# Aedelon/ProteinBERT-PyTorch-Replication

Measured on AMD Instinct MI355X. Metric: sequences/sec (whole node) ProteinBERT pretrain L=512 at 1/2/4/8 MI355X, higher is better.
Workload: dtype bf16; 1 GPU; global_batch=2048, per_gpu_batch=2048, seq_len=512, parallelism=dp1, impl=hip, hip_graph=False

## Files before the change

proteinbert_pytorch_replication_amd/ops/csrc/ln.hip:

```cpp
#include "mfma.h"
#include <stdlib.h>

using namespace pbx;
typedef unsigned short bf16_t;

namespace {
constexpr int CH = 128;
constexpr int BML = 32;

__device__ __forceinline__ void load_f8(const float* p, float* v) {
  const float4 a = *reinterpret_cast<const float4*>(p);
  const float4 c = *reinterpret_cast<const float4*>(p + 4);
  v[0] = a.x; v[1] = a.y; v[2] = a.z; v[3] = a.w; v[4] = c.x; v[5] = c.y; v[6] = c.z; v[7] = c.w;
}

__device__ __forceinline__ void stage_weight(unsigned char* dst, const bf16_t* __restrict__ w, int rows) {
  stage_chunks(
      rows * 16, [&](int idx) { return *reinterpret_cast<const uint4*>(w + (size_t)idx * 8); },
      [&](int idx, uint4 v) { *reinterpret_cast<uint4*>(dst + swz256(idx >> 4, idx & 15)) = v; });
}

constexpr int PB = 32;
constexpr int YS = CH + 4;

__device__ __forceinline__ uint4 ldq(const bf16_t* p, bool ok) {
  return ok ? *reinterpret_cast<const uint4*>(p) : make_uint4(0u, 0u, 0u, 0u);
}

__device__ __forceinline__ void sample_stats(float* sh, const float* __restrict__ st, int T, int BM, int L, float eps,
                                             const float* __restrict__ sums, int Ts, float inv_n) {
  if (threadIdx.x == 0) {
    float mean, rstd;
    ln_stats(st, T, BM, L, CH, eps, mean, rstd);
    sh[0] = mean;
    sh[1] = rstd;
    if (sums != nullptr) {
      float m1, m2;
      ln_bwd_consts(sums, Ts, inv_n, m1, m2);
      sh[2] = m1;
      sh[3] = m2;
    }
  }
}

__global__ void __launch_bounds__(512) ln_linear_fwd_kernel(
    const bf16_t* __restrict__ s1, const float* __restrict__ st1, int T1, int BM1, const float* __restrict__ g1,
    const float* __restrict__ be1, const bf16_t* __restrict__ wl, const float* __restrict__ bl,
    bf16_t* __restrict__ pre_l, bf16_t* __restrict__ s2, float* __restrict__ st2, int B, int L, float eps) {
  extern __shared__ __attribute__((aligned(16))) unsigned char smem[];
  unsigned char* ws = smem;
  unsigned char* ht = smem + 32768;
  float* yt = reinterpret_cast<float*>(smem + 32768 + PB * 256);
  float* tab = yt + PB * YS;
  const int tid = threadIdx.x, lane = tid & 63, w = tid >> 6;
  const int r = lane & 31, h = lane >> 5;
  const int j = tid >> 4, ch = tid & 15;
  const int l0 = blockIdx.x * PB, l = l0 + j;
  const bool okl = l < L;
  const int TP = (L + PB - 1) / PB;
  const int nbg = gridDim.y;
  const int b0 = (int)((long)B * blockIdx.y / nbg), b1 = (int)((long)B * (blockIdx.y + 1) / nbg);
  const int nb = b1 - b0;
  float* part = tab + 2 * nb;
  stage_weight(ws, wl, CH);
  for (int i = w; i < nb; i += 8) {
    float mean, rstd;
    wave_ln_stats(st1 + (size_t)(b0 + i) * T1 * 2, T1, BM1, L, CH, eps, mean, rstd);
    if (lane == 0) {
      tab[2 * i] = mean;
      tab[2 * i + 1] = rstd;
    }
  }
  float gam[8] = {0, 0, 0, 0, 0, 0, 0, 0}, bet[8] = {0, 0, 0, 0, 0, 0, 0, 0}, bb[8];
  if (okl) {
    load_f8(g1 + (size_t)l * CH + ch * 8, gam);
    load_f8(be1 + (size_t)l * CH + ch * 8, bet);
  }
  load_f8(bl + ch * 8, bb);
  uint4 nxt = ldq(s1 + ((size_t)b0 * L + l) * CH + ch * 8, okl && nb > 0);
  __syncthreads();
  for (int b = b0; b < b1; ++b) {
    const int i = b - b0;
    const float mean = tab[2 * i], rstd = tab[2 * i + 1];
    float sv[8], h1[8];
    unpack8(nxt, sv);
#pragma unroll
    for (int e = 0; e < 8; ++e) h1[e] = okl ? (sv[e] - mean) * rstd * gam[e] + bet[e] : 0.f;
    *reinterpret_cast<uint4*>(ht + swz256(j, ch)) = packq8(h1);
    __syncthreads();
    nxt = ldq(s1 + ((size_t)(b + 1) * L + l) * CH + ch * 8, okl && b + 1 < b1);
    if (w < 4) {
      f32x16_t acc = zero16();
#pragma unroll
      for (int kk = 0; kk < 8; ++kk)
        acc = mfma32(lds_frag(ws, swz256(w * 32 + r, kk * 2 + h)), lds_frag(ht, swz256(r, kk * 2 + h)), acc);
#pragma unroll
      for (int g = 0; g < 4; ++g)
        *reinterpret_cast<float4*>(yt + r * YS + w * 32 + 8 * g + 4 * h) =
            make_float4(acc[4 * g], acc[4 * g + 1], acc[4 * g + 2], acc[4 * g + 3]);
    }
    __syncthreads();
    float pre[8], o[8];
    const float4 ya = *reinterpret_cast<const float4*>(yt + j * YS + ch * 8);
    const float4 yb = *reinterpret_cast<const float4*>(yt + j * YS + ch * 8 + 4);
    const float yv[8] = {ya.x, ya.y, ya.z, ya.w, yb.x, yb.y, yb.z, yb.w};
#pragma unroll
    for (int e = 0; e < 8; ++e) pre[e] = yv[e] + bb[e];
    f32x2 gg[4];
    {
      const f32x2 xi[4] = {(f32x2){pre[0], pre[1]}, (f32x2){pre[2], pre[3]}, (f32x2){pre[4], pre[5]},
                           (f32x2){pre[6], pre[7]}};
      gelu2_fast_n<4, false>(xi, gg);
    }
#pragma unroll
    for (int e = 0; e < 8; ++e) o[e] = h1[e] + ((e & 1) ? gg[e >> 1].y : gg[e >> 1].x);
    const uint4 oq = packq8(o);
    if (okl) {
      const size_t off = ((size_t)b * L + l) * CH + ch * 8;
      if (pre_l != nullptr) *reinterpret_cast<uint4*>(pre_l + off) = packq8(pre);
      *reinterpret_cast<uint4*>(s2 + off) = oq;
    }
    float orr[8];
    unpack8(oq, orr);
    float sa = 0.f, sq = 0.f;
#pragma unroll
    for (int e = 0; e < 8; ++e) {
      sa += orr[e];
      sq += orr[e] * orr[e];
    }
    sa = wave_reduce_sum(okl ? sa : 0.f);
    sq = wave_reduce_sum(okl ? sq : 0.f);
    if (lane == 0) { part[(i * 8 + w) * 2] = sa; part[(i * 8 + w) * 2 + 1] = sq; }
  }
  __syncthreads();
  const int vrows = min(PB, L - l0);
  for (int i = tid; i < nb; i += 512) {
    float sa = 0.f, sq = 0.f;
#pragma unroll
    for (int ww = 0; ww < 8; ++ww) {
      sa += part[(i * 8 + ww) * 2];
      sq += part[(i * 8 + ww) * 2 + 1];
    }
    const float m = sa / (float)(vrows * CH);
    st2[((size_t)(b0 + i) * TP + blockIdx.x) * 2] = m;
    st2[((size_t)(b0 + i) * TP + blockIdx.x) * 2 + 1] = fmaxf(sq - sa * m, 0.f);
  }
}

__global__ void __launch_bounds__(256) ln2_consts_kernel(const float* __restrict__ st2, int T2, int BM2,
                                                         const float* __restrict__ sums2, int TS2,
                                                         const float* __restrict__ st1, int T1, int BM1,
                                                         float* __restrict__ consts, float* __restrict__ zero128,
                                                         int B, int L, float eps) {
  const int b = blockIdx.x * 4 + (threadIdx.x >> 6);
  if (b >= B) return;
  if (zero128 != nullptr)
    *reinterpret_cast<float2*>(zero128 + (size_t)b * CH + 2 * (threadIdx.x & 63)) = make_float2(0.f, 0.f);
  float mean2, rstd2, m1, m2, mean1, rstd1;
  wave_ln_stats(st2 + (size_t)b * T2 * 2, T2, BM2, L, CH, eps, mean2, rstd2);
  wave_bwd_consts(sums2 + (size_t)b * TS2 * 2, TS2, 1.0f / (float)(L * CH), m1, m2);
  wave_ln_stats(st1 + (size_t)b * T1 * 2, T1, BM1, L, CH, eps, mean1, rstd1);
  if ((threadIdx.x & 63) == 0) {
    float4* c = reinterpret_cast<float4*>(consts + (size_t)b * 8);
    c[0] = make_float4(mean2, rstd2, m1, m2);
    c[1] = make_float4(mean1, rstd1, 0.f, 0.f);
  }
}

__global__ void __launch_bounds__(512) ln2_linear_bwd_kernel(
    const bf16_t* __restrict__ dh2, const bf16_t* __restrict__ s2, const float* __restrict__ g2,
    const bf16_t* __restrict__ pre_l, const bf16_t* __restrict__ s1,
    const float* __restrict__ g1, const float* __restrict__ be1, const bf16_t* __restrict__ wl,
    const float* __restrict__ consts,
    bf16_t* __restrict__ dh1, float* __restrict__ sums1, float* __restrict__ dg2, float* __restrict__ db2,
    float* __restrict__ dg1, float* __restrict__ db1, float* __restrict__ dwl, float* __restrict__ dbl,
    float* __restrict__ dwl_slab, float* __restrict__ dbl_slab, int B, int L) {
  extern __shared__ __attribute__((aligned(16))) unsigned char smem[];
  unsigned char* ws = smem;
  unsigned char* dt = smem + 32768;
  unsigned char* ht = dt + 32 * 256;
  float* yt = reinterpret_cast<float*>(ht + 32 * 256);
  const int tid = threadIdx.x, lane = tid & 63, w = tid >> 6;
  const int r = lane & 31, h = lane >> 5;
  const int q = tr_q(lane), tc = tr_c(lane);
  const int j = tid >> 4, ch = tid & 15;
  const int TS1 = (L + 1) / 2;
  const int nsplit = gridDim.y;
  const int b0 = (int)((long)B * blockIdx.y / nsplit), b1 = (int)((long)B * (blockIdx.y + 1) / nsplit);
  stage_weight(ws, wl, CH);
  float adbl[8] = {0, 0, 0, 0, 0, 0, 0, 0};
  f32x16_t aw0 = zero16(), aw1 = zero16();
  const int wco = (w >> 1) * 32, wci = (w & 1) * 64;
  for (int pair = blockIdx.x; pair < TS1; pair += gridDim.x) {
    const int l = pair * 2 + (j & 1);
    const bool okl = l < L;
    float ga2[8] = {0, 0, 0, 0, 0, 0, 0, 0}, ga1[8] = {0, 0, 0, 0, 0, 0, 0, 0}, bt1[8] = {0, 0, 0, 0, 0, 0, 0, 0};
    if (okl) {
      load_f8(g2 + (size_t)l * CH + ch * 8, ga2);
      load_f8(g1 + (size_t)l * CH + ch * 8, ga1);
      load_f8(be1 + (size_t)l * CH + ch * 8, bt1);
    }
    float adg2[8] = {0, 0, 0, 0, 0, 0, 0, 0}, adb2[8] = {0, 0, 0, 0, 0, 0, 0, 0};
    float adg1[8] = {0, 0, 0, 0, 0, 0, 0, 0}, adb1[8] = {0, 0, 0, 0, 0, 0, 0, 0};
    const size_t coff = (size_t)l * CH + ch * 8;
    int bs = b0 + (j >> 1);
    bool ok = okl && bs < b1;
    size_t off = (size_t)bs * L * CH + coff;
    uint4 n_dh = ldq(dh2 + off, ok), n_s2 = ldq(s2 + off, ok), n_s1 = ldq(s1 + off, ok);
    uint4 n_pr = ldq(pre_l + off, ok);
    float4 n_c0 = make_float4(0.f, 1.f, 0.f, 0.f), n_c1 = make_float4(0.f, 1.f, 0.f, 0.f);
    if (bs < b1) {
      n_c0 = *reinterpret_cast<const float4*>(consts + (size_t)bs * 8);
      n_c1 = *reinterpret_cast<const float4*>(consts + (size_t)bs * 8 + 4);
    }
    for (int bc = b0; bc < b1; bc += 16) {
      const int bcur = bs;
      const bool okc = ok;
      const size_t offc = off;
      const float mean2 = n_c0.x, rstd2 = n_c0.y, m1 = n_c0.z, m2 = n_c0.w, mean1 = n_c1.x, rstd1 = n_c1.y;
      float dh[8], sv2[8], pr[8], sv1[8], ds2[8], dp[8], xh1[8], hv[8];
      unpack8(n_dh, dh);
      unpack8(n_s2, sv2);
      unpack8(n_s1, sv1);
#pragma unroll
      for (int e = 0; e < 8; ++e) {
        const float xh2 = (sv2[e] - mean2) * rstd2;
        adg2[e] += okc ? dh[e] * xh2 : 0.f;
        adb2[e] += okc ? dh[e] : 0.f;
        ds2[e] = okc ? rstd2 * (dh[e] * ga2[e] - m1 - xh2 * m2) : 0.f;
        xh1[e] = (sv1[e] - mean1) * rstd1;
        hv[e] = okc ? xh1[e] * ga1[e] + bt1[e] : 0.f;
      }
      *reinterpret_cast<uint4*>(ht + swz256(j, ch)) = packq8(hv);
      auto prefetch = [&]() {
        bs = bc + 16 + (j >> 1);
        ok = okl && bs < b1;
        off = (size_t)bs * L * CH + coff;
        n_dh = ldq(dh2 + off, ok);
        n_s2 = ldq(s2 + off, ok);
        n_pr = ldq(pre_l + off, ok);
        n_s1 = ldq(s1 + off, ok);
        if (bs < b1) {
          n_c0 = *reinterpret_cast<const float4*>(consts + (size_t)bs * 8);
          n_c1 = *reinterpret_cast<const float4*>(consts + (size_t)bs * 8 + 4);
        }
      };
      unpack8(n_pr, pr);
      float gp[8];
      {
        const f32x2 xi[4] = {(f32x2){pr[0], pr[1]}, (f32x2){pr[2], pr[3]}, (f32x2){pr[4], pr[5]},
                             (f32x2){pr[6], pr[7]}};
        f32x2 go[4];
        gelu2_fast_n<4, true>(xi, go);
#pragma unroll
        for (int e = 0; e < 4; ++e) {
          gp[2 * e] = go[e].x;
          gp[2 * e + 1] = go[e].y;
        }
      }
#pragma unroll
      for (int e = 0; e < 8; ++e) dp[e] = ds2[e] * gp[e];
      const uint4 dq = packq8(dp);
      *reinterpret_cast<uint4*>(dt + swz256(j, ch)) = dq;
      {
        float dpr[8];
        unpack8(dq, dpr);
#pragma unroll
        for (int e = 0; e < 8; ++e) adbl[e] += dpr[e];
      }
      __syncthreads();
      prefetch();
      if (w < 4) {
        f32x16_t acc = zero16();
#pragma unroll
        for (int kk = 0; kk < 8; ++kk) {
          const int rlo = kk * 16 + 8 * h + q;
          const int col = w * 32 + tc;
          const bf16x8 fa = cat_tr(lds_tr(ws, swz256e(rlo, col)), lds_tr(ws, swz256e(rlo + 4, col)));
          acc = mfma32(fa, lds_frag(dt, swz256(r, kk * 2 + h)), acc);
        }
#pragma unroll
        for (int g = 0; g < 4; ++g)
          *reinterpret_cast<float4*>(yt + r * YS + w * 32 + 8 * g + 4 * h) =
              make_float4(acc[4 * g], acc[4 * g + 1], acc[4 * g + 2], acc[4 * g + 3]);
      }
#pragma unroll
      for (int ks = 0; ks < 2; ++ks) {
        const int rlo = ks * 16 + 8 * h + q;
        const bf16x8 fa = cat_tr(lds_tr(dt, swz256e(rlo, wco + tc)), lds_tr(dt, swz256e(rlo + 4, wco + tc)));
        const bf16x8 fb0 = cat_tr(lds_tr(ht, swz256e(rlo, wci + tc)), lds_tr(ht, swz256e(rlo + 4, wci + tc)));
        const bf16x8 fb1 =
            cat_tr(lds_tr(ht, swz256e(rlo, wci + 32 + tc)), lds_tr(ht, swz256e(rlo + 4, wci + 32 + tc)));
        aw0 = mfma32(fa, fb0, aw0);
        aw1 = mfma32(fa, fb1, aw1);
      }
      __syncthreads();
      const float4 ya = *reinterpret_cast<const float4*>(yt + j * YS + ch * 8);
      const float4 yb = *reinterpret_cast<const float4*>(yt + j * YS + ch * 8 + 4);
      const float yv[8] = {ya.x, ya.y, ya.z, ya.w, yb.x, yb.y, yb.z, yb.w};
      float o[8], sa = 0.f, sc = 0.f;
#pragma unroll
      for (int e = 0; e < 8; ++e) {
        o[e] = okc ? bfround(ds2[e] + yv[e]) : 0.f;
        const float dxh = o[e] * ga1[e];
        sa += dxh;
        sc += dxh * xh1[e];
        adg1[e] += o[e] * xh1[e];
        adb1[e] += o[e];
      }
      if (okc) *reinterpret_cast<uint4*>(dh1 + offc) = packq8(o);
#pragma unroll
      for (int m = 1; m <= 16; m <<= 1) {
        sa += __shfl_xor(sa, m, 64);
        sc += __shfl_xor(sc, m, 64);
      }
      if ((lane & 31) == 0 && bcur < b1) {
        sums1[((size_t)bcur * TS1 + pair) * 2] = sa;
        sums1[((size_t)bcur * TS1 + pair) * 2 + 1] = sc;
      }
    }
    const int l0 = pair * 2;
    float* accs[4] = {adg2, adb2, adg1, adb1};
    float* dsts[4] = {dg2, db2, dg1, db1};
#pragma unroll
    for (int a = 0; a < 4; ++a) {
      __syncthreads();
#pragma unroll
      for (int e = 0; e < 8; ++e) yt[j * CH + ch * 8 + e] = accs[a][e];
      __syncthreads();
      if (tid < 2 * CH) {
        const int par = tid >> 7, c = tid & (CH - 1);
        float v = 0.f;
#pragma unroll
        for (int k = 0; k < 16; ++k) v += yt[(2 * k + par) * CH + c];
        if (l0 + par < L) atomicAdd(dsts[a] + (size_t)(l0 + par) * CH + c, v);
      }
    }
    __syncthreads();
  }
  __syncthreads();
#pragma unroll
  for (int e = 0; e < 8; ++e) yt[j * CH + ch * 8 + e] = adbl[e];
  __syncthreads();
  if (tid < CH) {
    float a = 0.f;
#pragma unroll 8
    for (int k = 0; k < 32; ++k) a += yt[k * CH + tid];
    if (dbl_slab != nullptr) dbl_slab[(size_t)(blockIdx.y * gridDim.x + blockIdx.x) * CH + tid] = a;
    else atomicAdd(dbl + tid, a);
  }
  float* dw = dwl_slab != nullptr ? dwl_slab + (size_t)(blockIdx.y * gridDim.x + blockIdx.x) * CH * CH : dwl;
#pragma unroll
  for (int i = 0; i < 16; ++i) {
    const int co = wco + (i & 3) + 8 * (i >> 2) + 4 * h;
    if (dwl_slab != nullptr) {
      dw[(size_t)co * CH + wci + r] = aw0[i];
      dw[(size_t)co * CH + wci + 32 + r] = aw1[i];
    } else {
      atomicAdd(dw + (size_t)co * CH + wci + r, aw0[i]);
      atomicAdd(dw + (size_t)co * CH + wci + 32 + r, aw1[i]);
    }
  }
}

__global__ void __launch_bounds__(512) ln1_finalize_kernel(
    const bf16_t* __restrict__ dh1, const bf16_t* __restrict__ s1, const float* __restrict__ st1, int T1, int BM1,
    const float* __restrict__ sums1, int TS1, const float* __restrict__ g1, bf16_t* __restrict__ ds1,
    float* __restrict__ dgb, int B, int L, float eps) {
  extern __shared__ __attribute__((aligned(16))) unsigned char smem[];
  float* red = reinterpret_cast<float*>(smem);
  float* tab = red + 2 * PB * CH;
  const int tid = threadIdx.x, lane = tid & 63, w = tid >> 6;
  const int j = tid >> 4, ch = tid & 15;
  const int nbg = gridDim.y;
  const int b0 = (int)((long)B * blockIdx.y / nbg), b1 = (int)((long)B * (blockIdx.y + 1) / nbg);
  const int nb = b1 - b0;
  float* dacc = tab + 4 * nb;
  const float inv_n = 1.0f / (float)(L * CH);
  for (int i = w; i < nb; i += 8) {
    float mean, rstd, m1, m2;
    wave_ln_stats(st1 + (size_t)(b0 + i) * T1 * 2, T1, BM1, L, CH, eps, mean, rstd);
    wave_bwd_consts(sums1 + (size_t)(b0 + i) * TS1 * 2, TS1, inv_n, m1, m2);
    if (lane == 0) { tab[4 * i] = mean; tab[4 * i + 1] = rstd; tab[4 * i + 2] = m1; tab[4 * i + 3] = m2; }
  }
  for (int i = tid; i < nb * CH; i += 512) dacc[i] = 0.f;
  const int TP = (L + PB - 1) / PB;
  int it = 0;
  for (int px = blockIdx.x; px < TP; px += gridDim.x) {
    const int l = px * PB + j;
    const bool okl = l < L;
    float ga[8] = {0, 0, 0, 0, 0, 0, 0, 0};
    if (okl) load_f8(g1 + (size_t)l * CH + ch * 8, ga);
    const size_t coff = (size_t)min(l, L - 1) * CH + ch * 8;
    uint4 n_dh = *reinterpret_cast<const uint4*>(dh1 + (size_t)min(b0, B - 1) * L * CH + coff);
    uint4 n_s = *reinterpret_cast<const uint4*>(s1 + (size_t)min(b0, B - 1) * L * CH + coff);
    __syncthreads();
    for (int b = b0; b < b1; ++b, ++it) {
      const float* tb = tab + 4 * (b - b0);
      const float mean = tb[0], rstd = tb[1], m1 = tb[2], m2 = tb[3];
      float* rb = red + (it & 1) * PB * CH;
      float dv[8], sv[8], o[8];
      unpack8(n_dh, dv);
      unpack8(n_s, sv);
      const size_t noff = (size_t)min(b + 1, B - 1) * L * CH + coff;
      n_dh = *reinterpret_cast<const uint4*>(dh1 + noff);
      n_s = *reinterpret_cast<const uint4*>(s1 + noff);
#pragma unroll
      for (int e = 0; e < 8; ++e) o[e] = okl ? rstd * (dv[e] * ga[e] - m1 - (sv[e] - mean) * rstd * m2) : 0.f;
      const uint4 qv = packq8(o);
      if (okl) *reinterpret_cast<uint4*>(ds1 + (size_t)b * L * CH + (size_t)l * CH + ch * 8) = qv;
      unpack8(qv, o);
#pragma unroll
      for (int e = 0; e < 8; ++e) {
        o[e] += __shfl_xor(o[e], 16, 64);
        o[e] += __shfl_xor(o[e], 32, 64);
      }
      if (lane < 16) {
        *reinterpret_cast<float4*>(rb + w * CH + ch * 8) = make_float4(o[0], o[1], o[2], o[3]);
        *reinterpret_cast<float4*>(rb + w * CH + ch * 8 + 4) = make_float4(o[4], o[5], o[6], o[7]);
      }
      __syncthreads();
      if (tid < CH) {
        float a = 0.f;
#pragma unroll
        for (int k = 0; k < 8; ++k) a += rb[k * CH + tid];
        dacc[(b - b0) * CH + tid] += a;
      }
    }
  }
  __syncthreads();
  for (int i = tid; i < nb * CH; i += 512) atomicAdd(dgb + (size_t)(b0 + i / CH) * CH + i % CH, dacc[i]);
}

__global__ void __launch_bounds__(256) embed_fwd_kernel(const long long* __restrict__ tok, const float* __restrict__ E,
                                                        bf16_t* __restrict__ out, long rows) {
  const long i = (long)blockIdx.x * 256 + threadIdx.x;
  if (i >= rows * 16) return;
  const long row = i >> 4;
  const int c8 = (int)(i & 15);
  const long long t = tok[row];
  float v[8];
  load_f8(E + (size_t)t * CH + c8 * 8, v);
  *reinterpret_cast<uint4*>(out + row * CH + c8 * 8) = packq8(v);
}

template <bool DPRE>
__global__ void __launch_bounds__(256) embed_bwd_kernel(const long long* __restrict__ tok,
                                                        const bf16_t* __restrict__ dout, float* __restrict__ dE,
                                                        long rows, int V, float* __restrict__ slab,
                                                        const bf16_t* __restrict__ gdn, const bf16_t* __restrict__ gdw,
                                                        bf16_t* __restrict__ dpn, bf16_t* __restrict__ dpw) {
  __shared__ __attribute__((aligned(16))) unsigned char ds[256 * 256];
  __shared__ int ts[256];
  const int tid = threadIdx.x, lane = tid & 63, w = tid >> 6;
  const int r = lane & 31, h = lane >> 5;
  const int q = tr_q(lane), tc = tr_c(lane);
  const long per = (rows + gridDim.x - 1) / gridDim.x;
  const long r0 = (long)blockIdx.x * per, r1 = min(rows, r0 + per);
  f32x16_t acc = zero16();
  for (long t0 = r0; t0 < r1; t0 += 256) {
    const int n = (int)min((long)256, r1 - t0);
    __syncthreads();
    if constexpr (DPRE) {
      for (int base = tid; base < 256 * 16; base += 4 * 256) {
        uint4 gq[4], nq[4], wq[4];
#pragma unroll
        for (int i = 0; i < 4; ++i) {
          const int idx = base + i * 256, row = idx >> 4;
          const size_t off = (size_t)(t0 + min(row, n - 1)) * CH + (idx & 15) * 8;
          gq[i] = *reinterpret_cast<const uint4*>(dout + off);
          nq[i] = *reinterpret_cast<const uint4*>(gdn + off);
          wq[i] = *reinterpret_cast<const uint4*>(gdw + off);
        }
#pragma unroll
        for (int i = 0; i < 4; ++i) {
          const int idx = base + i * 256, row = idx >> 4;
          const bool ok = row < n;
          *reinterpret_cast<uint4*>(ds + swz256(row, idx & 15)) = ok ? gq[i] : make_uint4(0u, 0u, 0u, 0u);
          if (ok) {
            float g[8], pn[8], pw[8], on[8], ow[8];
            unpack8(gq[i], g);
            unpack8(nq[i], pn);
            unpack8(wq[i], pw);
#pragma unroll
            for (int e = 0; e < 8; ++e) {
              on[e] = pn[e] * g[e];
              ow[e] = pw[e] * g[e];
            }
            const size_t off = (size_t)(t0 + row) * CH + (idx & 15) * 8;
            *reinterpret_cast<uint4*>(dpn + off) = packq8(on);
            *reinterpret_cast<uint4*>(dpw + off) = packq8(ow);
          }
        }
      }
    } else {
      stage_chunks(
          256 * 16,
          [&](int idx) {
            const int row = idx >> 4;
            return row < n ? *reinterpret_cast<const uint4*>(dout + (t0 + row) * CH + (idx & 15) * 8)
                           : make_uint4(0u, 0u, 0u, 0u);
          },
          [&](int idx, uint4 v) { *reinterpret_cast<uint4*>(ds + swz256(idx >> 4, idx & 15)) = v; });
    }
    ts[tid] = tid < n ? (int)tok[t0 + tid] : -1;
    __syncthreads();
    const int colb = w * 32 + tc;
#pragma unroll 4
    for (int kb = 0; kb < 16; ++kb) {
      typedef __attribute__((ext_vector_type(8))) unsigned short u16x8;
      u16x8 oh;
#pragma unroll
      for (int j = 0; j < 8; ++j) oh[j] = ts[kb * 16 + 8 * h + j] == r ? (unsigned short)0x3F80 : (unsigned short)0;
      const int rb = kb * 16 + 8 * h + q;
      const bf16x8 fb = cat_tr(lds_tr(ds, swz256e(rb, colb)), lds_tr(ds, swz256e(rb + 4, colb)));
      acc = mfma32(__builtin_bit_cast(bf16x8, oh), fb, acc);
    }
  }
#pragma unroll
  for (int i = 0; i < 16; ++i) {
    const int v = (i & 3) + 8 * (i >> 2) + 4 * h;
    if (slab != nullptr) {
      if (v < V) slab[((size_t)blockIdx.x * V + v) * CH + w * 32 + r] = acc[i];
    } else if (v < V && acc[i] != 0.f) {
      atomicAdd(dE + v * CH + w * 32 + r, acc[i]);
    }
  }
}

int g_cus = -1;
int num_cus() {
  if (g_cus < 0) {
    int dev = 0;
    g_cus = 256;
    if (hipGetDevice(&dev) == hipSuccess) {
      hipDeviceProp_t p;
      if (hipGetDeviceProperties(&p, dev) == hipSuccess) g_cus = p.multiProcessorCount;
    }
  }
  return g_cus;
}
int persistent_grid(int tiles, int per_cu) {
  const int cap = num_cus() * per_cu;
  return tiles < cap ? (tiles > 0 ? tiles : 1) : cap;
}
}

extern "C" int pbx_colsum_add(const float* src, int rows, int cols, float* dst, const float* scale, hipStream_t st);

static bool ln_attrs_set = false;
static void set_ln_attrs() {
  if (ln_attrs_set) return;
  (void)hipFuncSetAttribute((const void*)ln_linear_fwd_kernel, hipFuncAttributeMaxDynamicSharedMemorySize, 163840);
  (void)hipFuncSetAttribute((const void*)ln2_linear_bwd_kernel, hipFuncAttributeMaxDynamicSharedMemorySize, 163840);
  (void)hipFuncSetAttribute((const void*)ln1_finalize_kernel, hipFuncAttributeMaxDynamicSharedMemorySize, 163840);
  ln_attrs_set = true;
}

static int ln_groups(int B, int L) {
  const int tp = (L + PB - 1) / PB;
  int g = (2 * num_cus() + tp - 1) / tp;
  return g < 1 ? 1 : (g > B ? B : g);
}

PBX_EXPORT int pbx_ln_linear_fwd(const void* s1, const float* st1, int T1, int BM1, const float* g1,
                                 const float* be1, const void* wl, const float* bl, void* pre_l, void* s2,
                                 float* st2, int B, int L, float eps, hipStream_t st) {
  dim3 grid((L + PB - 1) / PB, ln_groups(B, L));
  const int nbmax = (B + (int)grid.y - 1) / (int)grid.y;
  const int lds = 32768 + PB * 256 + PB * YS * 4 + nbmax * 18 * 4;
  if (lds > 163840) return (int)hipErrorInvalidValue;
  set_ln_attrs();
  hipLaunchKernelGGL(ln_linear_fwd_kernel, grid, dim3(512), lds, st, (const bf16_t*)s1, st1, T1, BM1, g1, be1,
                     (const bf16_t*)wl, bl, (bf16_t*)pre_l, (bf16_t*)s2, st2, B, L, eps);
  return pbx_launch_status();
}

static void ln2_bwd_grid(int B, int L, int det, int& gx, int& nsplit) {
  const int pairs = (L + 1) / 2;
  const int target = num_cus();
  nsplit = (target + pairs - 1) / pairs;
  if (nsplit > (B + 15) / 16) nsplit = (B + 15) / 16;
  if (nsplit < 1 || det) nsplit = 1;
  gx = pairs < target ? pairs : target;
}

PBX_EXPORT int pbx_ln2_bwd_slab_rows(int B, int L, int det) {
  int gx, nsplit;
  ln2_bwd_grid(B, L, det, gx, nsplit);
  return gx * nsplit;
}

PBX_EXPORT int pbx_ln2_linear_bwd(const void* dh2, const void* s2, const float* st2, const float* sums2, int TS2,
                                  const float* g2, const void* pre_l, const void* s1, const float* st1, int T1,
                                  int BM1, const float* g1, const float* be1, const void* wl, float* consts,
                                  void* dh1, float* sums1, float* dg2, float* db2, float* dg1, float* db1, float* dwl,
                                  float* dbl, float* dgb_zero, int B, int L, float eps, float* dwl_slab, int slab_rows,
                                  int det, int fold, int consts_ready, hipStream_t st) {
  set_ln_attrs();
  const int T2 = (L + PB - 1) / PB;
  if (!consts_ready)
    hipLaunchKernelGGL(ln2_consts_kernel, dim3((B + 3) / 4), dim3(256), 0, st, st2, T2, PB, sums2, TS2, st1, T1, BM1,
                       consts, dgb_zero, B, L, eps);
  int gx, nsplit;
  ln2_bwd_grid(B, L, det, gx, nsplit);
  const int lds = 32768 + 2 * 32 * 256 + 32 * YS * 4;
  const int nwg = gx * nsplit;
  float* slab = dwl_slab != nullptr && nwg <= slab_rows ? dwl_slab : nullptr;
  float* bslab = slab != nullptr ? slab + (size_t)slab_rows * CH * CH : nullptr;
  if ((det || !fold) && slab == nullptr) return (int)hipErrorInvalidValue;
  hipLaunchKernelGGL(ln2_linear_bwd_kernel, dim3(gx, nsplit), dim3(512), lds, st, (const bf16_t*)dh2,
                     (const bf16_t*)s2, g2, (const bf16_t*)pre_l, (const bf16_t*)s1, g1, be1, (const bf16_t*)wl,
                     consts, (bf16_t*)dh1, sums1, dg2, db2, dg1, db1, dwl, dbl, slab, bslab, B, L);
  if (slab != nullptr && fold) {
    int rc = pbx_launch_status();
    if (rc != 0) return rc;
    rc = pbx_colsum_add(slab, nwg, CH * CH, dwl, nullptr, st);
    if (rc != 0) return rc;
    return pbx_colsum_add(bslab, nwg, CH, dbl, nullptr, st);
  }
  return pbx_launch_status();
}

PBX_EXPORT int pbx_ln1_finalize(const void* dh1, const void* s1, const float* st1, int T1, int BM1,
                                const float* sums1, int TS1, const float* g1, void* ds1, float* dgb, int B, int L,
                                float eps, int det, hipStream_t st) {
  const int tp = (L + PB - 1) / PB;
  const int gx = det ? 1 : (tp < 16 ? tp : 16);
  int gy = (2 * num_cus() + gx - 1) / gx;
  gy = gy < 1 ? 1 : (gy > B ? B : gy);
  dim3 grid(gx, gy);
  const int nbmax = (B + (int)grid.y - 1) / (int)grid.y;
  const int lds = 2 * PB * CH * 4 + nbmax * 16 + nbmax * CH * 4;
  if (lds > 163840) return (int)hipErrorInvalidValue;
  set_ln_attrs();
  hipLaunchKernelGGL(ln1_finalize_kernel, grid, dim3(512), lds, st, (const bf16_t*)dh1, (const bf16_t*)s1, st1, T1,
                     BM1, sums1, TS1, g1, (bf16_t*)ds1, dgb, B, L, eps);
  return pbx_launch_status();
}

PBX_EXPORT int pbx_embed_fwd(const void* tok, const float* E, void* out, long rows, hipStream_t st) {
  const long n = rows * 16;
  hipLaunchKernelGGL(embed_fwd_kernel, dim3((unsigned)((n + 255) / 256)), dim3(256), 0, st, (const long long*)tok, E,
                     (bf16_t*)out, rows);
  return pbx_launch_status();
}

PBX_EXPORT int pbx_embed_bwd_groups(long rows) {
  long g = (rows + 511) / 512;
  if (g > 2 * num_cus()) g = 2 * num_cus();
  return g < 1 ? 1 : (int)g;
}

PBX_EXPORT int pbx_embed_bwd(const void* tok, const void* dout, float* dE, long rows, int V, float* slab,
                             hipStream_t st) {
  if (V > 32) return (int)hipErrorInvalidValue;
  const int g = pbx_embed_bwd_groups(rows);
  hipLaunchKernelGGL(embed_bwd_kernel<false>, dim3((unsigned)g), dim3(256), 0, st, (const long long*)tok,
                     (const bf16_t*)dout, dE, rows, V, slab, nullptr, nullptr, nullptr, nullptr);
  if (slab != nullptr) {
    const int rc = pbx_launch_status();
    if (rc != 0) return rc;
    return pbx_colsum_add(slab, g, V * CH, dE, nullptr, st);
  }
  return pbx_launch_status();
}

PBX_EXPORT int pbx_embed_dpre(const void* tok, const void* ds1, const void* gdn, const void* gdw, void* dpn, void* dpw,
                              float* dE, long rows, int V, float* slab, hipStream_t st) {
  if (V > 32 || rows < 1) return (int)hipErrorInvalidValue;
  const int g = pbx_embed_bwd_groups(rows);
  hipLaunchKernelGGL(embed_bwd_kernel<true>, dim3((unsigned)g), dim3(256), 0, st, (const long long*)tok,
                     (const bf16_t*)ds1, dE, rows, V, slab, (const bf16_t*)gdn, (const bf16_t*)gdw, (bf16_t*)dpn,
                     (bf16_t*)dpw);
  if (slab != nullptr) {
    const int rc = pbx_launch_status();
    if (rc != 0) return rc;
    return pbx_colsum_add(slab, g, V * CH, dE, nullptr, st);
  }
  return pbx_launch_status();
}
```

Before: 108,800 sequences/s.

## Stream ln2 backward inputs through an LDS ring with direct global-to-LDS loads

Replaces the register-held one-step prefetch of dh2/s2/pre_l/s1 and the per-sample constants in the ln2+linear backward kernel with a two-deep per-wave LDS ring. The ring is filled by global_load_lds_dwordx4 issued two iterations ahead, with manual vmcnt waits. Out-of-range lanes read from a zero buffer. The aim is to hide global load latency and cut register pressure, at the cost of 80 KB extra LDS per workgroup, which may lower occupancy. Hand-placed waitcnt assembly risks ordering bugs.

After: 108,600 sequences/s. No clear change (-0.1%).

```diff
diff --git a/proteinbert_pytorch_replication_amd/ops/csrc/ln.hip b/proteinbert_pytorch_replication_amd/ops/csrc/ln.hip
--- a/proteinbert_pytorch_replication_amd/ops/csrc/ln.hip
+++ b/proteinbert_pytorch_replication_amd/ops/csrc/ln.hip
@@ -26,6 +26,25 @@
 __device__ __forceinline__ uint4 ldq(const bf16_t* p, bool ok) {
   return ok ? *reinterpret_cast<const uint4*>(p) : make_uint4(0u, 0u, 0u, 0u);
 }
+
+__device__ __attribute__((aligned(16))) unsigned int g_zero16_ln[4];
+
+__device__ __forceinline__ void glds16_ln(const void* src, unsigned char* lds_base) {
+  const unsigned dst = __builtin_amdgcn_readfirstlane(
+      (unsigned)(size_t)(__attribute__((address_space(3))) unsigned char*)lds_base);
+  unsigned keep;
+  asm volatile("s_mov_b32 %0, m0\n\ts_mov_b32 m0, %2\n\ts_nop 0\n\tglobal_load_lds_dwordx4 %1, off\n\ts_mov_b32 m0, %0"
+               : "=&s"(keep)
+               : "v"(src), "s"(dst)
+               : "memory");
+}
+
+constexpr int RING_T = 5;
+constexpr int RING_WAVE = RING_T * 1024;
+constexpr int RING_SLOT = 8 * RING_WAVE;
+constexpr int RING_DEPTH = 2;
+constexpr int LN2_BWD_LDS = 32768 + 2 * 32 * 256 + 32 * YS * 4 + RING_DEPTH * RING_SLOT;
+static_assert(LN2_BWD_LDS <= 163840, "LDS");
 
 __device__ __forceinline__ void sample_stats(float* sh, const float* __restrict__ st, int T, int BM, int L, float eps,
                                              const float* __restrict__ sums, int Ts, float inv_n) {
@@ -180,10 +199,13 @@
   unsigned char* dt = smem + 32768;
   unsigned char* ht = dt + 32 * 256;
   float* yt = reinterpret_cast<float*>(ht + 32 * 256);
-  const int tid = threadIdx.x, lane = tid & 63, w = tid >> 6;
+  const int tid = threadIdx.x, lane = tid & 63, w = __builtin_amdgcn_readfirstlane(tid >> 6);
   const int r = lane & 31, h = lane >> 5;
   const int q = tr_q(lane), tc = tr_c(lane);
   const int j = tid >> 4, ch = tid & 15;
+  unsigned char* ring = reinterpret_cast<unsigned char*>(yt + 32 * YS) + w * RING_WAVE;
+  unsigned long zero = (unsigned long)g_zero16_ln;
+  asm volatile("" : "+s"(zero));
   const int TS1 = (L + 1) / 2;
   const int nsplit = gridDim.y;
   const int b0 = (int)((long)B * blockIdx.y / nsplit), b1 = (int)((long)B * (blockIdx.y + 1) / nsplit);
@@ -203,20 +225,41 @@
     float adg2[8] = {0, 0, 0, 0, 0, 0, 0, 0}, adb2[8] = {0, 0, 0, 0, 0, 0, 0, 0};
     float adg1[8] = {0, 0, 0, 0, 0, 0, 0, 0}, adb1[8] = {0, 0, 0, 0, 0, 0, 0, 0};
     const size_t coff = (size_t)l * CH + ch * 8;
-    int bs = b0 + (j >> 1);
-    bool ok = okl && bs < b1;
-    size_t off = (size_t)bs * L * CH + coff;
-    uint4 n_dh = ldq(dh2 + off, ok), n_s2 = ldq(s2 + off, ok), n_s1 = ldq(s1 + off, ok);
-    uint4 n_pr = ldq(pre_l + off, ok);
-    float4 n_c0 = make_float4(0.f, 1.f, 0.f, 0.f), n_c1 = make_float4(0.f, 1.f, 0.f, 0.f);
-    if (bs < b1) {
-      n_c0 = *reinterpret_cast<const float4*>(consts + (size_t)bs * 8);
-      n_c1 = *reinterpret_cast<const float4*>(consts + (size_t)bs * 8 + 4);
-    }
-    for (int bc = b0; bc < b1; bc += 16) {
-      const int bcur = bs;
-      const bool okc = ok;
-      const size_t offc = off;
+#pragma unroll
+    for (int e = 0; e < 8; ++e) asm volatile("" : "+v"(ga2[e]), "+v"(ga1[e]), "+v"(bt1[e]));
+    auto issue = [&](int t) {
+      unsigned char* dst = ring + (t & 1) * RING_SLOT;
+      const int bt = b0 + 16 * t;
+      const bool ok = okl && bt + (j >> 1) < b1;
+      unsigned long o = ((unsigned long)(bt + (j >> 1)) * L * CH + coff) * 2;
+      asm volatile("" : "+v"(o));
+      glds16_ln((const void*)(ok ? (unsigned long)dh2 + o : zero), dst);
+      glds16_ln((const void*)(ok ? (unsigned long)s2 + o : zero), dst + 1024);
+      glds16_ln((const void*)(ok ? (unsigned long)pre_l + o : zero), dst + 2048);
+      glds16_ln((const void*)(ok ? (unsigned long)s1 + o : zero), dst + 3072);
+      const int bsc = bt + 2 * w + ((lane >> 1) & 1);
+      unsigned long oc = (unsigned long)bsc * 32 + (lane & 1) * 16;
+      asm volatile("" : "+v"(oc));
+      glds16_ln((const void*)(bsc < b1 ? (unsigned long)consts + oc : zero), dst + 4096);
+    };
+    const int nt = (b1 - b0 + 15) >> 4;
+    issue(0);
+    issue(1);
+    asm volatile("s_waitcnt vmcnt(%0)" ::"n"(RING_T) : "memory");
+    for (int t = 0; t < nt; ++t) {
+      const int bc = b0 + 16 * t;
+      const int bcur = bc + (j >> 1);
+      const bool okc = okl && bcur < b1;
+      const size_t offc = (size_t)bcur * L * CH + coff;
+      const unsigned char* sl = ring + (t & 1) * RING_SLOT;
+      const uint4 n_dh = *reinterpret_cast<const uint4*>(sl + lane * 16);
+      const uint4 n_s2 = *reinterpret_cast<const uint4*>(sl + 1024 + lane * 16);
+      const uint4 n_pr = *reinterpret_cast<const uint4*>(sl + 2048 + lane * 16);
+      const uint4 n_s1 = *reinterpret_cast<const uint4*>(sl + 3072 + lane * 16);
+      const float4 n_c0 = *reinterpret_cast<const float4*>(sl + 4096 + (lane >> 5) * 32);
+      const float4 n_c1 = *reinterpret_cast<const float4*>(sl + 4096 + (lane >> 5) * 32 + 16);
+      asm volatile("s_waitcnt lgkmcnt(0)" ::: "memory");
+      issue(t + 2);
       const float mean2 = n_c0.x, rstd2 = n_c0.y, m1 = n_c0.z, m2 = n_c0.w, mean1 = n_c1.x, rstd1 = n_c1.y;
       float dh[8], sv2[8], pr[8], sv1[8], ds2[8], dp[8], xh1[8], hv[8];
       unpack8(n_dh, dh);
@@ -232,19 +275,6 @@
         hv[e] = okc ? xh1[e] * ga1[e] + bt1[e] : 0.f;
       }
       *reinterpret_cast<uint4*>(ht + swz256(j, ch)) = packq8(hv);
-      auto prefetch = [&]() {
-        bs = bc + 16 + (j >> 1);
-        ok = okl && bs < b1;
-        off = (size_t)bs * L * CH + coff;
-        n_dh = ldq(dh2 + off, ok);
-        n_s2 = ldq(s2 + off, ok);
-        n_pr = ldq(pre_l + off, ok);
-        n_s1 = ldq(s1 + off, ok);
-        if (bs < b1) {
-          n_c0 = *reinterpret_cast<const float4*>(consts + (size_t)bs * 8);
-          n_c1 = *reinterpret_cast<const float4*>(consts + (size_t)bs * 8 + 4);
-        }
-      };
       unpack8(n_pr, pr);
       float gp[8];
       {
@@ -269,7 +299,6 @@
         for (int e = 0; e < 8; ++e) adbl[e] += dpr[e];
       }
       __syncthreads();
-      prefetch();
       if (w < 4) {
         f32x16_t acc = zero16();
 #pragma unroll
@@ -308,6 +337,7 @@
         adg1[e] += o[e] * xh1[e];
         adb1[e] += o[e];
       }
+      asm volatile("s_waitcnt vmcnt(%0)" ::"n"(RING_T) : "memory");
       if (okc) *reinterpret_cast<uint4*>(dh1 + offc) = packq8(o);
 #pragma unroll
       for (int m = 1; m <= 16; m <<= 1) {
@@ -319,6 +349,7 @@
         sums1[((size_t)bcur * TS1 + pair) * 2 + 1] = sc;
       }
     }
+    asm volatile("s_waitcnt vmcnt(0)" ::: "memory");
     const int l0 = pair * 2;
     float* accs[4] = {adg2, adb2, adg1, adb1};
     float* dsts[4] = {dg2, db2, dg1, db1};
@@ -604,7 +635,7 @@
                        consts, dgb_zero, B, L, eps);
   int gx, nsplit;
   ln2_bwd_grid(B, L, det, gx, nsplit);
-  const int lds = 32768 + 2 * 32 * 256 + 32 * YS * 4;
+  const int lds = LN2_BWD_LDS;
   const int nwg = gx * nsplit;
   float* slab = dwl_slab != nullptr && nwg <= slab_rows ? dwl_slab : nullptr;
   float* bslab = slab != nullptr ? slab + (size_t)slab_rows * CH * CH : nullptr;
```
